# janosh/torch-mnf

Measured on NVIDIA B200. Metric: flow log-prob points/s, higher is better.
Workload: dtype f32

## Files before the change

torch-mnf_b200/csrc/flow_pl.cu:

```cuda
#include "flow_math.cuh"
#include "tc_common.cuh"

namespace mnf {
namespace fpl {
using tc::smem_u32; using tc::mbar_init; using tc::mbar_arrive; using tc::mbar_wait; using tc::bulk_load;

constexpr int PMAX = 511;
constexpr int BP_FLOATS = 512;
constexpr int MAX_GROUPS = 2 * MNF_MAX_OPS;
constexpr int HDR_INTS = 4;
constexpr int HDR_FLOATS = MAX_GROUPS * HDR_INTS;
constexpr int MAX_H = 64;
constexpr double FAST_T = 32.0;
constexpr float FAST_B_MAX = 32.f;
constexpr int NB_MIN = 64, NB_MAX = 2048;
constexpr int SMEM_TABLE_FLOATS = 216 * 1024 / 4;
constexpr double LOG2E_D = 1.4426950408889634;

__host__ __device__ constexpr int round4i(int n) { return (n + 3) / 4 * 4; }
__host__ __device__ constexpr int nsf_doff(int K) { return 4 * K; }
__host__ __device__ constexpr int nsf_org(int K) { return 4 * K + round4i(2 * (K - 1)); }
__host__ __device__ constexpr int nsf_stride4(int K) { return (nsf_org(K) / 4 + 1) | 1; }
constexpr int AFF_ORG = 4, AFF_STRIDE4 = 3;
__host__ __device__ constexpr int region_floats(int stride4) { return BP_FLOATS + (PMAX + 1) * 4 * stride4; }

struct GroupList {
    int n;
    int region[MAX_GROUPS];
    unsigned char op[MAX_GROUPS];
    unsigned char which[MAX_GROUPS];
    signed char group_of[MNF_MAX_OPS][2];
};

__device__ __forceinline__ int bucket_of(float c, float lo, float inv, float nbm1) {
    const float t = fminf(fmaxf((c - lo) * inv, 0.f), nbm1);
    return __float_as_int(__fadd_rz(t, 8388608.f)) & 0x7fffff;
}

constexpr int BW = 8;

__device__ int envelope_line(const double *A, const double *B, int o0, int K, double lo, double hi) {
    int l = o0;
    if (lo == -INFINITY || hi == INFINITY) {
        const double sg = lo == -INFINITY ? -1.0 : 1.0;
        for (int k = o0 + 1; k < o0 + K; ++k)
            if (sg * A[k] > sg * A[l] || (A[k] == A[l] && B[k] > B[l])) l = k;
    } else {
        const double m = 0.5 * lo + 0.5 * hi;
        for (int k = o0 + 1; k < o0 + K; ++k)
            if (fma(A[k], m, B[k]) > fma(A[l], m, B[l])) l = k;
    }
    return l;
}

__device__ double envelope_gap(const double *A, const double *B, int K, double lo, double hi, double e) {
    double g = 0.0;
    for (int o0 = 0; o0 < 2 * K; o0 += K) {
        const int l = envelope_line(A, B, o0, K, lo, hi);
        const double vl = fma(A[l], e, B[l]);
        for (int k = o0; k < o0 + K; ++k) g = fmax(g, fma(A[k], e, B[k]) - vl);
    }
    return g;
}

__device__ bool split_piece(const double *A, const double *B, int K, double lo, double hi, double *out, int *cnt) {
    const double TN = FAST_T / LOG2E_D;
    auto emit = [&](double s) {
        const int p = atomicAdd(cnt, 1);
        if (p < PMAX) out[p] = s;
        return p < PMAX;
    };
    double seg[2][2] = {{lo, hi}, {0.0, 0.0}};
    int nseg = 1;
    if (lo == -INFINITY && hi == INFINITY) {
        if (!emit(0.0)) return false;
        seg[0][1] = 0.0, seg[1][0] = 0.0, seg[1][1] = INFINITY, nseg = 2;
    }
    for (int q = 0; q < nseg; ++q) {
        double a = seg[q][0], b = seg[q][1];
        const bool left = a == -INFINITY, right = b == INFINITY;
        if (left || right) {
            const double e = left ? b : a;
            if (envelope_gap(A, B, K, a, b, e) <= TN) continue;
            double w = fmax(1.0, fabs(e)), s;
            for (;;) {
                s = (double)(float)(left ? e - w : e + w);
                if (fabs(s) > 1.0e38) return false;
                if (envelope_gap(A, B, K, left ? -INFINITY : s, left ? s : INFINITY, s) <= TN) break;
                w *= 2.0;
            }
            if (!emit(s)) return false;
            a = left ? s : e, b = left ? e : s;
        }
        double st[64][2];
        int sp = 0;
        st[sp][0] = a, st[sp][1] = b, ++sp;
        while (sp) {
            --sp;
            const double x0 = st[sp][0], x1 = st[sp][1];
            if (envelope_gap(A, B, K, x0, x1, x0) <= TN && envelope_gap(A, B, K, x0, x1, x1) <= TN) continue;
            const double s = (double)(float)(0.5 * x0 + 0.5 * x1);
            if (!(s > x0 && s < x1) || sp + 2 > 64 || !emit(s)) return false;
            st[sp][0] = s, st[sp][1] = x1, ++sp;
            st[sp][0] = x0, st[sp][1] = s, ++sp;
        }
    }
    return true;
}

__device__ __forceinline__ double piece_point(const double *bp, int n, int i, double &lo, double &hi) {
    lo = i > 0 ? bp[i - 1] : -INFINITY;
    hi = i < n ? bp[i] : INFINITY;
    if (n == 0) return 0.0;
    if (i == 0) return hi - 1.0 - fabs(hi);
    if (i == n) return lo + 1.0 + fabs(lo);
    return 0.5 * lo + 0.5 * hi;
}

__device__ int net_pre_maps(const float *__restrict__ net, const int *sizes, int upto, double m, double (*va)[MNF_MAX_HIDDEN],
                            double (*vb)[MNF_MAX_HIDDEN], int lane) {
    const double slope_neg = (double)0.2f;
    int cur = 0;
    if (lane == 0) va[0][0] = 1.0, vb[0][0] = 0.0;
    __syncwarp();
    const float *p = net;
    for (int t = 0; t <= upto; ++t) {
        const int n_in = sizes[t], n_out = sizes[t + 1];
        const float *bias = p + n_in * n_out;
        for (int k = lane; k < n_out; k += 32) {
            double A = 0.0, B = (double)bias[k];
            const float *w = p + (size_t)k * n_in;
            for (int j = 0; j < n_in; ++j) {
                const double wj = (double)w[j];
                A = fma(wj, va[cur][j], A);
                B = fma(wj, vb[cur][j], B);
            }
            if (t < upto) {
                const double s = fma(A, m, B) > 0.0 ? 1.0 : slope_neg;
                A *= s, B *= s;
            }
            va[cur ^ 1][k] = A, vb[cur ^ 1][k] = B;
        }
        __syncwarp();
        cur ^= 1;
        p += n_in * n_out + n_out;
    }
    return cur;
}

__global__ void __launch_bounds__(32 * BW) flow_pl_build_kernel(const __grid_constant__ FlowProgram prog, const __grid_constant__ GroupList gl,
                                                                const float *__restrict__ params, float *__restrict__ image) {
    __shared__ double s_bp[512], s_tmp[512];
    __shared__ double s_va[BW][2][MNF_MAX_HIDDEN], s_vb[BW][2][MNF_MAX_HIDDEN];
    __shared__ int s_bidx[PMAX];
    __shared__ int s_n, s_ncand, s_fail;
    const int g = blockIdx.x, tid = threadIdx.x, warp = tid >> 5, lane = tid & 31, nt = blockDim.x;
    auto sort_bp = [&](int tot) {
        for (int e = tid; e < tot; e += nt) {
            const double v = s_bp[e];
            int r = 0;
            for (int u = 0; u < tot; ++u) r += (s_bp[u] < v || (s_bp[u] == v && u < e)) ? 1 : 0;
            s_tmp[r] = v;
        }
        __syncthreads();
        for (int e = tid; e < tot; e += nt) s_bp[e] = s_tmp[e];
        __syncthreads();
    };
    const mnf_flow_op &op = prog.ops[gl.op[g]];
    const bool nsf = op.type == MNF_OP_NSF_CL;
    const int K = op.K, L = op.n_lin, n_out = op.sizes[L];
    int n_nets = 0, net_off[2], net_slot[2];
    if (nsf) {
        net_off[0] = op.net_off[gl.which[g]], net_slot[0] = 0, n_nets = 1;
    } else {
        if (op.flags & MNF_FLAG_SCALE) net_off[n_nets] = op.net_off[0], net_slot[n_nets++] = 0;
        if (op.flags & MNF_FLAG_SHIFT) net_off[n_nets] = op.net_off[1], net_slot[n_nets++] = 1;
    }
    if (tid == 0) s_n = 0, s_ncand = 0;
    __syncthreads();

    bool over = false;
    for (int l = 1; l < L; ++l) {
        const int n = s_n;
        for (int i = warp; i <= n; i += BW) {
            double lo, hi;
            const double m = piece_point(s_bp, n, i, lo, hi);
            for (int q = 0; q < n_nets; ++q) {
                const int cur = net_pre_maps(params + net_off[q], op.sizes, l - 1, m, s_va[warp], s_vb[warp], lane);
                for (int k = lane; k < op.sizes[l]; k += 32) {
                    const double a = s_va[warp][cur][k], b = s_vb[warp][cur][k];
                    if (a != 0.0) {
                        const double tz = -b / a;
                        if (tz > lo && tz < hi && fabs(tz) < 3.0e38) {
                            const int pos = atomicAdd(&s_ncand, 1);
                            if (pos < 512) s_tmp[pos] = tz;
                        }
                    }
                }
                __syncwarp();
            }
        }
        __syncthreads();
        const int nc = s_ncand, tot = n + nc;
        if (tot > PMAX) {
            over = true;
            break;
        }
        for (int e = tid; e < nc; e += nt) s_bp[n + e] = s_tmp[e];
        __syncthreads();
        sort_bp(tot);
        if (tid == 0) s_n = tot, s_ncand = 0;
        __syncthreads();
    }

    float *region = image + gl.region[g];
    int *hdr = reinterpret_cast<int *>(image) + g * HDR_INTS;
    const int n = over ? 0 : s_n;
    if (tid == 0) hdr[0] = n, hdr[1] = over ? 1 : 0, hdr[2] = 0, hdr[3] = 0;
    for (int e = tid; e < BP_FLOATS; e += nt) region[e] = e < n ? (float)s_bp[e] : INFINITY;
    if (over) return;
    const int stride = 4 * (nsf ? nsf_stride4(K) : AFF_STRIDE4);
    auto write_rows = [&](int nn, float *rows, bool fast) {
        for (int i = warp; i <= nn; i += BW) {
            double lo, hi;
            const double m = piece_point(s_bp, nn, i, lo, hi);
            const float org = nn == 0 ? 0.f : (float)(i == 0 ? s_bp[0] : s_bp[i - 1]);
            float *row = rows + (size_t)i * stride;
            for (int e = lane; e < stride; e += 32) row[e] = 0.f;
            __syncwarp();
            for (int q = 0; q < n_nets; ++q) {
                const int cur = net_pre_maps(params + net_off[q], op.sizes, L - 1, m, s_va[warp], s_vb[warp], lane);
                const double *va = s_va[warp][cur], *vb = s_vb[warp][cur];
                for (int o = lane; o < n_out; o += 32) {
                    double A = va[o], B = vb[o], sc = 1.0;
                    if (fast && nsf) {
                        sc = LOG2E_D;
                        if (o < 2 * K) {
                            const int l = envelope_line(va, vb, o < K ? 0 : K, K, lo, hi);
                            A -= va[l], B -= vb[l];
                        }
                    }
                    const double V = fma(A, (double)org, B);
                    int ia, iv;
                    if (!nsf) ia = net_slot[q], iv = 2 + net_slot[q];
                    else if (o < 2 * K) ia = 4 * (o >> 1) + (o & 1), iv = ia + 2;
                    else ia = nsf_doff(K) + 2 * (o - 2 * K), iv = ia + 1;
                    row[ia] = (float)(A * sc), row[iv] = (float)(V * sc);
                }
                __syncwarp();
            }
            if (lane == 0) row[nsf ? nsf_org(K) : AFF_ORG] = org;
        }
    };
    write_rows(n, region + BP_FLOATS, false);

    __syncthreads();
    if (tid == 0) s_ncand = 0, s_fail = nsf && !(op.bound <= FAST_B_MAX);
    __syncthreads();
    if (nsf && !s_fail) {
        for (int i = warp; i <= n; i += BW) {
            double lo, hi;
            const double m = piece_point(s_bp, n, i, lo, hi);
            const int cur = net_pre_maps(params + net_off[0], op.sizes, L - 1, m, s_va[warp], s_vb[warp], lane);
            if (lane == 0 && !split_piece(s_va[warp][cur], s_vb[warp][cur], K, lo, hi, s_tmp, &s_ncand)) s_fail = 1;
            __syncwarp();
        }
    }
    __syncthreads();
    const int nf = n + s_ncand;
    if (s_fail || nf > PMAX) return;
    for (int e = tid; e < nf - n; e += nt) s_bp[n + e] = s_tmp[e];
    __syncthreads();
    sort_bp(nf);
    const int fast_off = BP_FLOATS + (n + 1) * stride, rows_floats = (nf + 1) * stride;
    const int budget = min((PMAX - n) * stride, SMEM_TABLE_FLOATS / gl.n);
    int nb = NB_MIN;
    float lo32 = 0.f, inv = 0.f;
    for (bool found = false; !found; nb *= 2) {
        if (nb > NB_MAX || 4 + 4 * nb + rows_floats > budget) return;
        for (int ab = 0; ab < 9 && !found; ++ab) {
            const int a = ab / 3, b = ab % 3;
            if (nf && a + b >= nf) continue;
            lo32 = nf ? (float)s_bp[a] : 0.f;
            const float hi32 = nf ? (float)s_bp[nf - 1 - b] : 0.f;
            inv = hi32 > lo32 ? (float)((double)nb / ((double)hi32 - (double)lo32)) : 0.f;
            for (int e = tid; e < nf; e += nt) s_bidx[e] = bucket_of((float)s_bp[e], lo32, inv, (float)(nb - 1));
            __syncthreads();
            int bad = 0;
            for (int e = tid; e + 3 < nf; e += nt) bad |= s_bidx[e] == s_bidx[e + 3];
            found = !__syncthreads_or(bad);
        }
        if (found) break;
    }
    float *fast = region + fast_off;
    for (int j = tid; j < nb; j += nt) {
        int a = 0, b = nf;
        while (a < b) {
            const int mid = (a + b) >> 1;
            if (s_bidx[mid] < j) a = mid + 1; else b = mid;
        }
        float4 r;
        r.x = __int_as_float(a);
        r.y = a < nf && s_bidx[a] == j ? (float)s_bp[a] : INFINITY;
        r.z = a + 1 < nf && s_bidx[a + 1] == j ? (float)s_bp[a + 1] : INFINITY;
        r.w = a + 2 < nf && s_bidx[a + 2] == j ? (float)s_bp[a + 2] : INFINITY;
        reinterpret_cast<float4 *>(fast)[1 + j] = r;
    }
    if (tid == 0) {
        fast[0] = lo32, fast[1] = inv, fast[2] = (float)(nb - 1), fast[3] = __int_as_float(4 + 4 * nb);
        hdr[2] = fast_off, hdr[3] = 4 + 4 * nb + rows_floats;
    }
    write_rows(nf, fast + 4 + 4 * nb, true);
}

struct Params {
    FlowProgram prog;
    GroupList gl;
    const float *params, *x, *image;
    float *y, *log_det, *base_lp, *inter;
    long long n_rows;
    int dir_flags, smem_floats;
    mnf_gather_out gather;
};

__device__ __forceinline__ float2 f2_fma(float2 a, float2 b, float2 c) {
    unsigned long long ra = *reinterpret_cast<unsigned long long *>(&a), rb = *reinterpret_cast<unsigned long long *>(&b),
                       rc = *reinterpret_cast<unsigned long long *>(&c), rd;
    asm("fma.rn.f32x2 %0, %1, %2, %3;" : "=l"(rd) : "l"(ra), "l"(rb), "l"(rc));
    return *reinterpret_cast<float2 *>(&rd);
}

__device__ __noinline__ void mlp_fp32(const float *__restrict__ net, int n_lin, const int *sizes, float c, float *out) {
    float h[2][MAX_H];
    h[0][0] = c;
    int cur = 0;
    const float *p = net;
    for (int t = 0; t < n_lin; ++t) {
        const int n_in = sizes[t], n_o = sizes[t + 1];
        for (int k = 0; k < n_o; ++k) {
            float acc = p[n_in * n_o + k];
            for (int j = 0; j < n_in; ++j) acc = fmaf(p[k * n_in + j], h[cur][j], acc);
            if (t + 1 < n_lin) h[cur ^ 1][k] = leaky02(acc);
            else out[k] = acc;
        }
        cur ^= 1;
        p += n_in * n_o + n_o;
    }
}

template <int K>
__device__ __noinline__ float2 nsf_fallback(const float *__restrict__ net, int n_lin, const int *sizes, float B, float edge_deriv, float c,
                                            bool inverse, float tr) {
    float raw[3 * K - 1], ld = 0.f;
    mlp_fp32(net, n_lin, sizes, c, raw);
    rq_spline<K, true>(raw, K, B, edge_deriv, inverse, tr, ld);
    return make_float2(tr, ld);
}
__device__ __noinline__ float mlp_fp32_scalar(const float *__restrict__ net, int n_lin, const int *sizes, float c) {
    float out[1];
    mlp_fp32(net, n_lin, sizes, c, out);
    return out[0];
}

template <int S>
__device__ __forceinline__ void search_steps(uint32_t &a, float c) {
    float t;
    asm("ld.shared.f32 %0, [%1+%2];" : "=f"(t) : "r"(a), "n"(4 * (S - 1)));
    if (c > t) a += 4u * S;
    if constexpr (S > 1) search_steps<S / 2>(a, c);
}

template <bool SM>
__device__ __forceinline__ int find_piece(const float *tb, float c) {
    if constexpr (SM) {
        const uint32_t base = smem_u32(tb);
        uint32_t a = base;
        search_steps<(PMAX + 1) / 2>(a, c);
        return (int)((a - base) >> 2);
    } else {
        int pos = 0;
#pragma unroll
        for (int s = (PMAX + 1) / 2; s >= 1; s >>= 1) pos += (c > tb[pos + s - 1]) ? s : 0;
        return pos;
    }
}

enum { KIND_PLAIN = 0, KIND_FAST = 1, KIND_OVER = 2 };

template <bool SM>
__device__ __forceinline__ const float4 *piece_row(const float *tb, bool fast, float c, int stride4) {
    if (fast) {
        const float4 gr = *reinterpret_cast<const float4 *>(tb);
        const float4 bk = reinterpret_cast<const float4 *>(tb)[1 + bucket_of(c, gr.x, gr.y, gr.z)];
        const int piece = __float_as_int(bk.x) + (c > bk.y) + (c > bk.z) + (c > bk.w);
        return reinterpret_cast<const float4 *>(tb + __float_as_int(gr.w)) + piece * stride4;
    }
    return reinterpret_cast<const float4 *>(tb + BP_FLOATS) + find_piece<SM>(tb, c) * stride4;
}

__device__ __forceinline__ float ex2_approx(float x) {
    float r;
    asm("ex2.approx.ftz.f32 %0, %1;" : "=f"(r) : "f"(x));
    return r;
}
__device__ __forceinline__ float sqrt_approx(float x) {
    float r;
    asm("sqrt.approx.ftz.f32 %0, %1;" : "=f"(r) : "f"(x));
    return r;
}
__device__ __forceinline__ float lg2_approx(float x) {
    float r;
    asm("lg2.approx.ftz.f32 %0, %1;" : "=f"(r) : "f"(x));
    return r;
}

constexpr float LOG2E = 1.4426950408889634f, LN2 = 0.6931471805599453f;

template <int K, bool FAST>
__device__ __forceinline__ void unit_knots(const float *raw, float twoB, float *tw, float *th) {
    constexpr float span = 1.f - kMinBin * (float)K;
    float ew[K], eh[K], sw = 0.f, sh = 0.f, scw, sch, offw, offh;
    if constexpr (FAST) {
#pragma unroll
        for (int k = 0; k < K; ++k) {
            ew[k] = ex2_approx(raw[k]), eh[k] = ex2_approx(raw[K + k]);
            sw += ew[k], sh += eh[k];
        }
        const float r = frcp<true>(sw * sh), s = twoB * LOG2E;
        scw = s * (r * sh), sch = s * (r * sw);
        offw = offh = -0.5f * s;
    } else {
        float mw = raw[0], mh = raw[K];
#pragma unroll
        for (int k = 1; k < K; ++k) mw = fmaxf(mw, raw[k]), mh = fmaxf(mh, raw[K + k]);
        const float mwn = -mw * LOG2E, mhn = -mh * LOG2E;
#pragma unroll
        for (int k = 0; k < K; ++k) {
            ew[k] = ex2_approx(fmaf(raw[k], LOG2E, mwn)), eh[k] = ex2_approx(fmaf(raw[K + k], LOG2E, mhn));
            sw += ew[k], sh += eh[k];
        }
        scw = twoB * frcp<true>(sw) * LOG2E, sch = twoB * frcp<true>(sh) * LOG2E;
        offw = twoB > 80.f ? -scw : 0.f, offh = twoB > 80.f ? -sch : 0.f;
    }
    float pw = 0.f, ph = 0.f;
#pragma unroll
    for (int k = 0; k < K; ++k) {
        pw += ex2_approx(fmaf(ew[k], scw, offw)), ph += ex2_approx(fmaf(eh[k], sch, offh));
        ew[k] = pw, eh[k] = ph;
    }
    float c1w, c1h;
    if constexpr (FAST) {
        const float r = frcp<true>(pw * ph);
        c1w = 2.f * span * (r * ph), c1h = 2.f * span * (r * pw);
    } else {
        c1w = 2.f * span * frcp<true>(pw), c1h = 2.f * span * frcp<true>(ph);
    }
    tw[0] = th[0] = -1.f;
#pragma unroll
    for (int k = 0; k + 1 < K; ++k) {
        tw[k + 1] = fmaf(ew[k], c1w, -1.f + 2.f * (float)(k + 1) * kMinBin);
        th[k + 1] = fmaf(eh[k], c1h, -1.f + 2.f * (float)(k + 1) * kMinBin);
    }
    tw[K] = th[K] = 1.f;
}

__device__ __forceinline__ float knot_derivative_log2(float r) {
    return fmaf(LN2, r > 20.f * LOG2E ? r : lg2_approx(2.f + ex2_approx(r)), kMinDeriv);
}

template <int K, bool FAST, class DerivFn>
__device__ __forceinline__ void rq_spline_lazy(const float *raw, float B, float inv_B, float edge_deriv, bool inverse, float &v, float &ld,
                                               DerivFn deriv) {
    float cw[K + 1], ch[K + 1];
    unit_knots<K, FAST>(raw, 2.f * B, cw, ch);
    const float u = v * inv_B;
    const float *sk = inverse ? ch : cw;
    int idx = 0;
    float xk = cw[0], xk1 = cw[1], yk = ch[0], yk1 = ch[1];
#pragma unroll
    for (int k = 1; k < K; ++k) {
        const bool ge = u >= sk[k];
        idx += ge ? 1 : 0;
        xk = ge ? cw[k] : xk, xk1 = ge ? cw[k + 1] : xk1;
        yk = ge ? ch[k] : yk, yk1 = ge ? ch[k + 1] : yk1;
    }
    const float wk = xk1 - xk, hk = yk1 - yk;
    const float r0 = deriv(max(idx - 1, 0)), r1 = deriv(min(idx, K - 2));
    float dk, dk1;
    if constexpr (FAST) {
        dk = (idx > 0) ? knot_derivative_log2(r0) : edge_deriv;
        dk1 = (idx < K - 1) ? knot_derivative_log2(r1) : edge_deriv;
    } else {
        dk = (idx > 0) ? knot_derivative<true>(r0) : edge_deriv;
        dk1 = (idx < K - 1) ? knot_derivative<true>(r1) : edge_deriv;
    }
    if (inverse) {
        const float dkw = dk * wk, dk1w = dk1 * wk;
        const float dsw = dkw + dk1w - 2.f * hk;
        const float dy = u - yk;
        const float a = dy * dsw + hk * (hk - dkw);
        const float b = hk * dkw - dy * dsw;
        const float c = -hk * dy;
        const float disc = fmaxf(b * b - 4.f * a * c, 0.f);
        const float root = __fdividef(2.f * c, -b - sqrt_approx(disc));
        v = (root * wk + xk) * B;
        const float tt = root * (1.f - root);
        const float omr = 1.f - root;
        const float den = wk * (hk + dsw * tt);
        const float num = (hk * hk) * wk * (dk1w * (root * root) + 2.f * hk * tt + dkw * (omr * omr));
        const float rd = frcp<true>(den);
        ld -= __logf(num * rd * rd);
    } else {
        const float sk_ = __fdividef(hk, wk);
        const float dsum = dk + dk1 - 2.f * sk_;
        const float th = __fdividef(u - xk, wk);
        const float tt = th * (1.f - th);
        const float numer = hk * (sk_ * (th * th) + dk * tt);
        const float den = sk_ + dsum * tt;
        const float omt = 1.f - th;
        const float num = (sk_ * sk_) * (dk1 * (th * th) + 2.f * sk_ * tt + dk * (omt * omt));
        const float rd = frcp<true>(den);
        v = fmaf(numer, rd, yk) * B;
        ld += __logf(num * rd * rd);
    }
}

constexpr int THREADS = 1024;

struct Exec {
    int type;
    int k;
    int g0, g1;
    int flag;
    int pad[3];
    float c[8];
};
static_assert(sizeof(Exec) == 64, "two 16-byte rows of ints, two of floats");

__device__ __forceinline__ void build_exec(const Params &p, Exec *ex, int *n_exec, int lane) {
    const int n = p.prog.n_ops, inverse = p.dir_flags & 1;
    if (lane < n) {
        const int k = inverse ? n - 1 - lane : lane;
        const mnf_flow_op &op = p.prog.ops[k];
        Exec e{};
        e.k = k;
        if (op.type == MNF_OP_AFFINE_CONST) {
            const double s0 = p.params[op.aux_off], s1 = p.params[op.aux_off + 1];
            const double t0 = p.params[op.aux_off + 2], t1 = p.params[op.aux_off + 3];
            if (inverse) {
                const double e0 = exp(-s0), e1 = exp(-s1);
                e.c[0] = (float)e0, e.c[3] = (float)e1, e.c[4] = (float)(-t0 * e0), e.c[5] = (float)(-t1 * e1), e.c[6] = (float)(-(s0 + s1));
            } else {
                e.c[0] = (float)exp(s0), e.c[3] = (float)exp(s1), e.c[4] = (float)t0, e.c[5] = (float)t1, e.c[6] = (float)(s0 + s1);
            }
        } else if (op.type == MNF_OP_GLOW) {
            const float *W = p.params + op.aux_off + (inverse ? 4 : 0);
            e.c[0] = W[0], e.c[1] = W[1], e.c[2] = W[2], e.c[3] = W[3];
            e.c[6] = inverse ? -p.params[op.aux_off + 8] : p.params[op.aux_off + 8];
        } else if (op.type == MNF_OP_AFFINE_HALF) {
            e.type = 1, e.g0 = p.gl.group_of[k][0], e.flag = (op.flags & MNF_FLAG_PARITY) ? 1 : 0;
        } else {
            e.type = 2, e.flag = inverse ? 0 : 1;
            e.g0 = p.gl.group_of[k][inverse ? 1 : 0], e.g1 = p.gl.group_of[k][inverse ? 0 : 1];
            e.c[0] = op.bound, e.c[1] = 1.f / op.bound, e.c[2] = op.edge_deriv;
        }
        ex[lane] = e;
    }
    __syncwarp();
    if (lane == 0) {
        int j = 0;
        bool open = false;
        double M[4], b[2], ld;
        for (int i = 0; i < n; ++i) {
            const Exec e = ex[i];
            if (e.type != 0 || p.inter) {
                ex[j++] = e, open = false;
                continue;
            }
            if (!open) {
                for (int q = 0; q < 4; ++q) M[q] = e.c[q];
                b[0] = e.c[4], b[1] = e.c[5], ld = e.c[6];
                ++j, open = true;
            } else {
                const double W0 = e.c[0], W1 = e.c[1], W2 = e.c[2], W3 = e.c[3];
                const double n00 = M[0] * W0 + M[1] * W2, n01 = M[0] * W1 + M[1] * W3;
                const double n10 = M[2] * W0 + M[3] * W2, n11 = M[2] * W1 + M[3] * W3;
                const double nb0 = b[0] * W0 + b[1] * W2 + e.c[4], nb1 = b[0] * W1 + b[1] * W3 + e.c[5];
                M[0] = n00, M[1] = n01, M[2] = n10, M[3] = n11, b[0] = nb0, b[1] = nb1, ld += e.c[6];
            }
            Exec f{};
            for (int q = 0; q < 4; ++q) f.c[q] = (float)M[q];
            f.c[4] = (float)b[0], f.c[5] = (float)b[1], f.c[6] = (float)ld;
            ex[j - 1] = f;
        }
        *n_exec = j;
    }
}

template <int K, bool SM>
__device__ __forceinline__ void run_points(const Params &p, const float *smem, const int *s_off, const int *s_goff, const int *s_kind,
                                           const Exec *ex, int n_exec) {
    const bool sum_lp = p.dir_flags & 2;
    auto table = [&](int g) -> const float * {
        if constexpr (SM) return smem + s_off[g];
        const int o = s_off[g];
        return o >= 0 ? smem + o : p.image + s_goff[g];
    };
    const long long stride = (long long)gridDim.x * blockDim.x;
#pragma unroll 1
    for (long long r = (long long)blockIdx.x * blockDim.x + threadIdx.x; r < p.n_rows; r += stride) {
        float v0, v1, ld = 0.f;
        {
            const float2 xin = ld_stream2(reinterpret_cast<const float2 *>(p.x) + r);
            v0 = xin.x, v1 = xin.y;
        }
#pragma unroll 1
        for (int kk = 0; kk < n_exec; ++kk) {
            const int4 ei = *reinterpret_cast<const int4 *>(&ex[kk]);
            if (ei.x == 0) {
                const float4 m = *reinterpret_cast<const float4 *>(ex[kk].c), b = *reinterpret_cast<const float4 *>(ex[kk].c + 4);
                const float n0 = fmaf(v1, m.z, fmaf(v0, m.x, b.x)), n1 = fmaf(v1, m.w, fmaf(v0, m.y, b.y));
                v0 = n0, v1 = n1, ld += b.z;
            } else if (ei.x == 1) {
                const mnf_flow_op &op = p.prog.ops[ei.y];
                const bool parity = ex[kk].flag != 0;
                const float c = parity ? v1 : v0;
                float tr = parity ? v0 : v1;
                const int g = ei.z;
                float s = 0.f, t = 0.f;
                if (g < 0) {
                } else if (s_kind[g] != KIND_OVER) {
                    const float4 *row = piece_row<SM>(table(g), s_kind[g] == KIND_FAST, c, AFF_STRIDE4);
                    const float4 q = row[0];
                    const float d = c - row[1].x;
                    s = fmaf(q.x, d, q.z), t = fmaf(q.y, d, q.w);
                } else {
                    if (op.flags & MNF_FLAG_SCALE) s = mlp_fp32_scalar(p.params + op.net_off[0], op.n_lin, op.sizes, c);
                    if (op.flags & MNF_FLAG_SHIFT) t = mlp_fp32_scalar(p.params + op.net_off[1], op.n_lin, op.sizes, c);
                }
                if (p.dir_flags & 1) {
                    tr = (tr - t) / expf(s), ld -= s;
                } else {
                    tr = expf(s) * tr + t, ld += s;
                }
                if (parity) v0 = tr; else v1 = tr;
            } else {
                const float4 cs = *reinterpret_cast<const float4 *>(ex[kk].c);
                const bool first_f1 = ex[kk].flag != 0;
#pragma unroll 1
                for (int step = 0; step < 2; ++step) {
                    const bool use_f1 = (step == 0) == first_f1;
                    const float c = use_f1 ? v0 : v1;
                    float tr = use_f1 ? v1 : v0;
                    const float B = cs.x;
                    if (tr >= -B && tr <= B) {
                        const int g = step ? ei.w : ei.z;
                        const int kind = s_kind[g];
                        if (kind != KIND_OVER) {
                            const float4 *row = piece_row<SM>(table(g), kind == KIND_FAST, c, nsf_stride4(K));
                            const float d = c - row[nsf_org(K) / 4].x;
                            const float2 dd = make_float2(d, d);
                            float raw[2 * K];
#pragma unroll
                            for (int j = 0; j < K; ++j) {
                                const float4 q = row[j];
                                const float2 o = f2_fma(make_float2(q.x, q.y), dd, make_float2(q.z, q.w));
                                raw[2 * j] = o.x, raw[2 * j + 1] = o.y;
                            }
                            const float2 *dv = reinterpret_cast<const float2 *>(row) + nsf_doff(K) / 2;
                            const auto deriv = [&](int j) {
                                const float2 q = dv[j];
                                return fmaf(q.x, d, q.y);
                            };
                            if (kind == KIND_FAST) rq_spline_lazy<K, true>(raw, B, cs.y, cs.z, (p.dir_flags & 1) != 0, tr, ld, deriv);
                            else rq_spline_lazy<K, false>(raw, B, cs.y, cs.z, (p.dir_flags & 1) != 0, tr, ld, deriv);
                        } else {
                            const mnf_flow_op &op = p.prog.ops[ei.y];
                            const float2 o = nsf_fallback<K>(p.params + op.net_off[use_f1 ? 0 : 1], op.n_lin, op.sizes, B, cs.z, c,
                                                             (p.dir_flags & 1) != 0, tr);
                            tr = o.x, ld += o.y;
                        }
                        if (use_f1) v1 = tr; else v0 = tr;
                    }
                }
            }
            if (p.inter) st_stream2(reinterpret_cast<float2 *>(p.inter + ((size_t)kk * p.n_rows + r) * 2), make_float2(v0, v1));
        }
        float lp = fmaf(-0.5f, fmaf(v0, v0, v1 * v1), -1.8378770664093453f);
        if (sum_lp) lp += ld;
        if (p.y) st_stream2(reinterpret_cast<float2 *>(p.y) + r, make_float2(v0, v1));
        if (p.log_det) p.log_det[r] = ld;
        if (p.base_lp) p.base_lp[r] = lp;
        if (p.gather.multicast_ptr) {
            asm volatile("multimem.st.relaxed.sys.global.f32 [%0], %1;" ::"l"(p.gather.multicast_ptr + p.gather.row_offset + r), "f"(lp)
                         : "memory");
        } else {
            for (int g = 0; g < p.gather.n_peers; ++g) p.gather.peer_ptrs[g][p.gather.row_offset + r] = lp;
        }
    }
}

template <int K>
__global__ void __launch_bounds__(THREADS, 1) flow_pl_kernel(const __grid_constant__ Params p) {
    extern __shared__ __align__(16) float smem[];
    __shared__ __align__(16) Exec s_exec[MNF_MAX_OPS];
    __shared__ int s_off[MAX_GROUPS], s_goff[MAX_GROUPS], s_kind[MAX_GROUPS];
    __shared__ int s_allfit, s_nexec;
    __shared__ __align__(8) unsigned long long s_bar;
    const int lane = threadIdx.x & 31, ng = p.gl.n;
    const uint32_t bar = smem_u32(&s_bar);
    if (threadIdx.x == 0) {
        mbar_init(bar, 1);
        asm volatile("fence.mbarrier_init.release.cluster;" ::: "memory");
    }
    __syncthreads();
    if (threadIdx.x >= 32 && threadIdx.x < 64) build_exec(p, s_exec, &s_nexec, lane);
    if (threadIdx.x < 32) {
        const int *hdr = reinterpret_cast<const int *>(p.image);
        int total = 0, fit = 1;
        for (int base = 0; base < ng; base += 32) {
            const int g = base + lane;
            int sz = 0, ov = 0, src = 0;
            if (g < ng) {
                const int4 h = *reinterpret_cast<const int4 *>(hdr + g * HDR_INTS);
                const int s4 = p.prog.ops[p.gl.op[g]].type == MNF_OP_NSF_CL ? nsf_stride4(K) : AFF_STRIDE4;
                ov = h.y;
                src = p.gl.region[g] + h.z;
                sz = ov ? 0 : h.z ? h.w : BP_FLOATS + (h.x + 1) * 4 * s4;
                s_kind[g] = ov ? KIND_OVER : h.z ? KIND_FAST : KIND_PLAIN;
                s_goff[g] = src;
            }
            int inc = sz;
#pragma unroll
            for (int o = 1; o < 32; o <<= 1) {
                const int t = __shfl_up_sync(0xffffffffu, inc, o);
                if (lane >= o) inc += t;
            }
            const int off = total + inc - sz;
            const bool ok = off + sz <= p.smem_floats;
            if (g < ng) {
                s_off[g] = (ov || !ok) ? -1 : off;
                if (!ov && ok) {
                    asm volatile("mbarrier.expect_tx.relaxed.cta.shared::cta.b64 [%0], %1;" ::"r"(bar), "r"((uint32_t)sz * 4u) : "memory");
                    bulk_load(smem_u32(smem + off), p.image + src, (uint32_t)sz * 4u, bar);
                }
            }
            fit &= __all_sync(0xffffffffu, g >= ng || ov || ok) ? 1 : 0;
            total += __shfl_sync(0xffffffffu, inc, 31);
        }
        __syncwarp();
        if (lane == 0) {
            s_allfit = fit;
            mbar_arrive(bar);
        }
    }
    __syncthreads();
    mbar_wait(bar, 0);
    if (s_allfit) run_points<K, true>(p, smem, s_off, s_goff, s_kind, s_exec, s_nexec);
    else run_points<K, false>(p, smem, s_off, s_goff, s_kind, s_exec, s_nexec);
}

#define MNF_PL_BINS(X) X(4) X(5) X(6) X(8) X(10) X(12) X(16)
constexpr int K_MAX = 16;
static bool k_instantiated(int K) {
#define MNF_PL_HAVE(KK) if (K == KK) return true;
    MNF_PL_BINS(MNF_PL_HAVE)
#undef MNF_PL_HAVE
    return false;
}

struct Plan {
    bool ok = false;
    int K = 8;
    GroupList gl;
    int64_t image_floats = 0;
};

static Plan make_plan(const mnf_flow_op *ops, int n_ops, int dim) {
    Plan pl;
    if (dim != 2 || n_ops < 1 || n_ops > MNF_MAX_OPS) return pl;
    int K = 0, n = 0;
    int64_t off = HDR_FLOATS;
    for (int k = 0; k < n_ops; ++k) {
        const mnf_flow_op &op = ops[k];
        pl.gl.group_of[k][0] = pl.gl.group_of[k][1] = -1;
        if (op.type == MNF_OP_AFFINE_CONST || op.type == MNF_OP_GLOW) continue;
        if (op.type != MNF_OP_AFFINE_HALF && op.type != MNF_OP_NSF_CL) return pl;
        if (op.n_lin < 2 || op.n_lin > MNF_MAX_LIN || op.sizes[0] != 1) return pl;
        for (int l = 1; l < op.n_lin; ++l)
            if (op.sizes[l] < 1 || op.sizes[l] > MAX_H) return pl;
        if (op.type == MNF_OP_NSF_CL) {
            if (!k_instantiated(op.K)) return pl;
            if (K && op.K != K) return pl;
            K = op.K;
            if (op.sizes[op.n_lin] != 3 * K - 1) return pl;
            for (int which = 0; which < 2; ++which) {
                pl.gl.group_of[k][which] = (signed char)n;
                pl.gl.op[n] = (unsigned char)k, pl.gl.which[n] = (unsigned char)which, pl.gl.region[n] = (int)off;
                off += region_floats(nsf_stride4(K));
                ++n;
            }
        } else {
            if (op.sizes[op.n_lin] != 1) return pl;
            if (!(op.flags & (MNF_FLAG_SCALE | MNF_FLAG_SHIFT))) continue;
            pl.gl.group_of[k][0] = (signed char)n;
            pl.gl.op[n] = (unsigned char)k, pl.gl.which[n] = 0, pl.gl.region[n] = (int)off;
            off += region_floats(AFF_STRIDE4);
            ++n;
        }
    }
    if (n == 0) return pl;
    pl.gl.n = n;
    pl.K = K ? K : 8;
    pl.image_floats = off;
    pl.ok = true;
    return pl;
}

template <int K>
static int launch_k(const Params &p, const DeviceProps *dp, size_t smem_bytes, cudaStream_t st) {
    static thread_local size_t attr_set[64] = {};
    int dev = 0;
    MNF_CUDA(cudaGetDevice(&dev));
    if (dev < 0 || dev >= 64 || attr_set[dev] < smem_bytes) {
        MNF_CUDA(cudaFuncSetAttribute(flow_pl_kernel<K>, cudaFuncAttributeMaxDynamicSharedMemorySize, (int)smem_bytes));
        if (dev >= 0 && dev < 64) attr_set[dev] = smem_bytes;
    }
    const int threads = p.n_rows <= (long long)dp->sm_count * 64 ? 64 : p.n_rows <= (long long)dp->sm_count * 256 ? 256 : THREADS;
    long long blocks = (p.n_rows + threads - 1) / threads;
    if (blocks > dp->sm_count) blocks = dp->sm_count;
    flow_pl_kernel<K><<<(unsigned)blocks, threads, smem_bytes, st>>>(p);
    return launch_status("flow_pl_kernel");
}

}

int64_t flow_pl_workspace_floats(int n_ops) {
    if (n_ops < 1) n_ops = 1;
    if (n_ops > MNF_MAX_OPS) n_ops = MNF_MAX_OPS;
    return fpl::HDR_FLOATS + (int64_t)2 * n_ops * fpl::region_floats(fpl::nsf_stride4(fpl::K_MAX));
}

int64_t flow_pl_image_floats(const mnf_flow_op *ops, int n_ops, int dim) {
    const fpl::Plan pl = fpl::make_plan(ops, n_ops, dim);
    return pl.ok ? pl.image_floats : 0;
}

int flow_pl_build(const mnf_flow_op *ops, int n_ops, const float *params, int dim, float *image, cudaStream_t stream) {
    using namespace fpl;
    const Plan pl = make_plan(ops, n_ops, dim);
    MNF_REQUIRE(pl.ok, MNF_E_SHAPE, "program has no piecewise-linear form");
    MNF_REQUIRE(params && image && ((uintptr_t)image % 16) == 0, MNF_E_ARG, "NULL or misaligned pointer");
    FlowProgram prog;
    prog.n_ops = n_ops;
    for (int k = 0; k < n_ops; ++k) prog.ops[k] = ops[k];
    flow_pl_build_kernel<<<pl.gl.n, 32 * BW, 0, stream>>>(prog, pl.gl, params, image);
    return launch_status("flow_pl_build_kernel");
}

int launch_flow_pl(const mnf_flow_op *ops, int n_ops, const float *params, const float *x, float *y, float *log_det,
                   float *base_lp, float *inter, int64_t n_rows, int dim, int dir_flags, float *workspace,
                   const mnf_gather_out *gather, cudaStream_t stream, bool plan_only) {
    using namespace fpl;
    const Plan pl = make_plan(ops, n_ops, dim);
    if (!pl.ok) return 1;
    if (plan_only) return 0;
    if (!workspace) return 1;
    const DeviceProps *dp = device_props();
    MNF_REQUIRE(dp != nullptr, MNF_E_DEVICE, "no CUDA device");
    MNF_REQUIRE(((uintptr_t)workspace % 16) == 0, MNF_E_ALIGN, "workspace must be 16-byte aligned");
    MNF_REQUIRE(((uintptr_t)x % 8) == 0 && (!y || ((uintptr_t)y % 8) == 0) && (!inter || ((uintptr_t)inter % 8) == 0), MNF_E_ALIGN,
                "x, y and intermediates must be 8-byte aligned");
    MNF_REQUIRE(n_rows > 0, MNF_E_ARG, "bad row count");
    if (!(dir_flags & 4)) {
        const int rc = flow_pl_build(ops, n_ops, params, dim, workspace, stream);
        if (rc) return rc;
    }
    Params p{};
    p.prog.n_ops = n_ops;
    for (int k = 0; k < n_ops; ++k) p.prog.ops[k] = ops[k];
    p.gl = pl.gl;
    p.params = params, p.x = x, p.image = workspace, p.y = y, p.log_det = log_det, p.base_lp = base_lp, p.inter = inter;
    p.n_rows = n_rows, p.dir_flags = dir_flags & 3;
    if (gather) {
        MNF_REQUIRE(gather->n_peers >= 0 && gather->n_peers <= MNF_MAX_PEERS, MNF_E_ARG, "bad n_peers");
        p.gather = *gather;
    }
    size_t want = (size_t)(pl.image_floats - HDR_FLOATS) * sizeof(float);
    const size_t cap = (size_t)dp->smem_optin - 4096;
    if (want > cap) want = cap;
    want &= ~(size_t)15;
    p.smem_floats = (int)(want / sizeof(float));
#define MNF_PL_LAUNCH(KK) if (pl.K == KK) return launch_k<KK>(p, dp, want, stream);
    MNF_PL_BINS(MNF_PL_LAUNCH)
#undef MNF_PL_LAUNCH
    return 1;
}

}
```

Measured before the change: 12.61 billion.

## Pack spline knot math into f32x2, defer log-det logs, template on direction

Reworks the rational-quadratic spline: width and height knot accumulation now uses paired f32x2 add/fma, and only the needed knot pair is reconstructed from cumulative sums instead of materialising full knot arrays. Per-spline log calls are replaced by a running mantissa/exponent product that is flushed with a single lg2 at the end or before fallback paths. Divisions become reciprocal multiplies, and the inverse flag becomes a template parameter so each kernel variant is specialised. This cuts MUFU and ALU work per point, at the cost of doubling kernel instantiations and a slight change in numeric rounding.

```diff
diff --git a/torch-mnf_b200/csrc/flow_pl.cu b/torch-mnf_b200/csrc/flow_pl.cu
--- a/torch-mnf_b200/csrc/flow_pl.cu
+++ b/torch-mnf_b200/csrc/flow_pl.cu
@@ -329,6 +329,12 @@
     asm("fma.rn.f32x2 %0, %1, %2, %3;" : "=l"(rd) : "l"(ra), "l"(rb), "l"(rc));
     return *reinterpret_cast<float2 *>(&rd);
 }
+__device__ __forceinline__ float2 f2_add(float2 a, float2 b) {
+    unsigned long long ra = *reinterpret_cast<unsigned long long *>(&a), rb = *reinterpret_cast<unsigned long long *>(&b), rd;
+    asm("add.rn.f32x2 %0, %1, %2;" : "=l"(rd) : "l"(ra), "l"(rb));
+    return *reinterpret_cast<float2 *>(&rd);
+}
+__device__ __forceinline__ float2 f2_splat(float a) { return make_float2(a, a); }
 
 __device__ __noinline__ void mlp_fp32(const float *__restrict__ net, int n_lin, const int *sizes, float c, float *out) {
     float h[2][MAX_H];
@@ -416,74 +422,87 @@
 
 constexpr float LOG2E = 1.4426950408889634f, LN2 = 0.6931471805599453f;
 
+__device__ __forceinline__ float knot_const(float k) { return fmaf(2.f * kMinBin, k, -1.f); }
+
 template <int K, bool FAST>
-__device__ __forceinline__ void unit_knots(const float *raw, float twoB, float *tw, float *th) {
+__device__ __forceinline__ void unit_knots(const float *raw, float twoB, float2 *S, float2 &c1) {
     constexpr float span = 1.f - kMinBin * (float)K;
-    float ew[K], eh[K], sw = 0.f, sh = 0.f, scw, sch, offw, offh;
+    float2 e[K], sc, off;
     if constexpr (FAST) {
+        float2 s1;
 #pragma unroll
         for (int k = 0; k < K; ++k) {
-            ew[k] = ex2_approx(raw[k]), eh[k] = ex2_approx(raw[K + k]);
-            sw += ew[k], sh += eh[k];
-        }
-        const float r = frcp<true>(sw * sh), s = twoB * LOG2E;
-        scw = s * (r * sh), sch = s * (r * sw);
-        offw = offh = -0.5f * s;
+            e[k] = make_float2(ex2_approx(raw[k]), ex2_approx(raw[K + k]));
+            s1 = k ? f2_add(s1, e[k]) : e[k];
+        }
+        const float r = frcp<true>(s1.x * s1.y), s = twoB * LOG2E;
+        sc = make_float2(s * (r * s1.y), s * (r * s1.x));
+        off = f2_splat(-0.5f * s);
     } else {
-        float mw = raw[0], mh = raw[K];
+        float mw = raw[0], mh = raw[K], sw = 0.f, sh = 0.f;
 #pragma unroll
         for (int k = 1; k < K; ++k) mw = fmaxf(mw, raw[k]), mh = fmaxf(mh, raw[K + k]);
         const float mwn = -mw * LOG2E, mhn = -mh * LOG2E;
 #pragma unroll
         for (int k = 0; k < K; ++k) {
-            ew[k] = ex2_approx(fmaf(raw[k], LOG2E, mwn)), eh[k] = ex2_approx(fmaf(raw[K + k], LOG2E, mhn));
-            sw += ew[k], sh += eh[k];
-        }
-        scw = twoB * frcp<true>(sw) * LOG2E, sch = twoB * frcp<true>(sh) * LOG2E;
-        offw = twoB > 80.f ? -scw : 0.f, offh = twoB > 80.f ? -sch : 0.f;
-    }
-    float pw = 0.f, ph = 0.f;
+            e[k] = make_float2(ex2_approx(fmaf(raw[k], LOG2E, mwn)), ex2_approx(fmaf(raw[K + k], LOG2E, mhn)));
+            sw += e[k].x, sh += e[k].y;
+        }
+        sc = make_float2(twoB * frcp<true>(sw) * LOG2E, twoB * frcp<true>(sh) * LOG2E);
+        off = make_float2(twoB > 80.f ? -sc.x : 0.f, twoB > 80.f ? -sc.y : 0.f);
+    }
+    float2 p;
 #pragma unroll
     for (int k = 0; k < K; ++k) {
-        pw += ex2_approx(fmaf(ew[k], scw, offw)), ph += ex2_approx(fmaf(eh[k], sch, offh));
-        ew[k] = pw, eh[k] = ph;
-    }
-    float c1w, c1h;
+        const float2 a = f2_fma(e[k], sc, off);
+        const float2 x = make_float2(ex2_approx(a.x), ex2_approx(a.y));
+        p = k ? f2_add(p, x) : x;
+        if (k + 1 < K) S[k] = p;
+    }
     if constexpr (FAST) {
-        const float r = frcp<true>(pw * ph);
-        c1w = 2.f * span * (r * ph), c1h = 2.f * span * (r * pw);
+        const float r = frcp<true>(p.x * p.y);
+        c1 = make_float2(2.f * span * (r * p.y), 2.f * span * (r * p.x));
     } else {
-        c1w = 2.f * span * frcp<true>(pw), c1h = 2.f * span * frcp<true>(ph);
-    }
-    tw[0] = th[0] = -1.f;
-#pragma unroll
-    for (int k = 0; k + 1 < K; ++k) {
-        tw[k + 1] = fmaf(ew[k], c1w, -1.f + 2.f * (float)(k + 1) * kMinBin);
-        th[k + 1] = fmaf(eh[k], c1h, -1.f + 2.f * (float)(k + 1) * kMinBin);
-    }
-    tw[K] = th[K] = 1.f;
+        c1 = make_float2(2.f * span * frcp<true>(p.x), 2.f * span * frcp<true>(p.y));
+    }
 }
 
 __device__ __forceinline__ float knot_derivative_log2(float r) {
     return fmaf(LN2, r > 20.f * LOG2E ? r : lg2_approx(2.f + ex2_approx(r)), kMinDeriv);
 }
 
-template <int K, bool FAST, class DerivFn>
-__device__ __forceinline__ void rq_spline_lazy(const float *raw, float B, float inv_B, float edge_deriv, bool inverse, float &v, float &ld,
+__device__ __forceinline__ void ld_mul(float &P, int &E, float q) {
+    P *= q;
+    const int eb = __float_as_int(P) & 0x7f800000;
+    E += (eb >> 23) - 127;
+    P *= __int_as_float(0x7f000000 - eb);
+}
+template <bool INV>
+__device__ __forceinline__ void ld_flush(float &ld, float &P, int &E) {
+    ld = fmaf(INV ? -LN2 : LN2, lg2_approx(P) + (float)E, ld);
+    P = 1.f, E = 0;
+}
+
+template <int K, bool FAST, bool INV, class DerivFn>
+__device__ __forceinline__ void rq_spline_lazy(const float *raw, float B, float inv_B, float edge_deriv, float &v, float &P, int &E,
                                                DerivFn deriv) {
-    float cw[K + 1], ch[K + 1];
-    unit_knots<K, FAST>(raw, 2.f * B, cw, ch);
+    float2 S[K - 1], c1;
+    unit_knots<K, FAST>(raw, 2.f * B, S, c1);
     const float u = v * inv_B;
-    const float *sk = inverse ? ch : cw;
     int idx = 0;
-    float xk = cw[0], xk1 = cw[1], yk = ch[0], yk1 = ch[1];
+    float2 lo = f2_splat(0.f), hi = S[0];
 #pragma unroll
     for (int k = 1; k < K; ++k) {
-        const bool ge = u >= sk[k];
+        const bool ge = u >= fmaf(INV ? S[k - 1].y : S[k - 1].x, INV ? c1.y : c1.x, knot_const((float)k));
         idx += ge ? 1 : 0;
-        xk = ge ? cw[k] : xk, xk1 = ge ? cw[k + 1] : xk1;
-        yk = ge ? ch[k] : yk, yk1 = ge ? ch[k + 1] : yk1;
-    }
+        lo = ge ? S[k - 1] : lo;
+        if (k + 1 < K) hi = ge ? S[k] : hi;
+    }
+    const float fidx = __int_as_float(0x4b000000 | idx) - 8388608.f;
+    const float k0 = knot_const(fidx), k1 = knot_const(fidx + 1.f);
+    const float xk = fmaf(lo.x, c1.x, k0), yk = fmaf(lo.y, c1.y, k0);
+    const bool last = idx == K - 1;
+    const float xk1 = last ? 1.f : fmaf(hi.x, c1.x, k1), yk1 = last ? 1.f : fmaf(hi.y, c1.y, k1);
     const float wk = xk1 - xk, hk = yk1 - yk;
     const float r0 = deriv(max(idx - 1, 0)), r1 = deriv(min(idx, K - 2));
     float dk, dk1;
@@ -494,7 +513,7 @@
         dk = (idx > 0) ? knot_derivative<true>(r0) : edge_deriv;
         dk1 = (idx < K - 1) ? knot_derivative<true>(r1) : edge_deriv;
     }
-    if (inverse) {
+    if constexpr (INV) {
         const float dkw = dk * wk, dk1w = dk1 * wk;
         const float dsw = dkw + dk1w - 2.f * hk;
         const float dy = u - yk;
@@ -502,18 +521,19 @@
         const float b = hk * dkw - dy * dsw;
         const float c = -hk * dy;
         const float disc = fmaxf(b * b - 4.f * a * c, 0.f);
-        const float root = __fdividef(2.f * c, -b - sqrt_approx(disc));
+        const float root = 2.f * c * frcp<true>(-b - sqrt_approx(disc));
         v = (root * wk + xk) * B;
         const float tt = root * (1.f - root);
         const float omr = 1.f - root;
         const float den = wk * (hk + dsw * tt);
         const float num = (hk * hk) * wk * (dk1w * (root * root) + 2.f * hk * tt + dkw * (omr * omr));
         const float rd = frcp<true>(den);
-        ld -= __logf(num * rd * rd);
+        ld_mul(P, E, num * rd * rd);
     } else {
-        const float sk_ = __fdividef(hk, wk);
+        const float rw = frcp<true>(wk);
+        const float sk_ = hk * rw;
         const float dsum = dk + dk1 - 2.f * sk_;
-        const float th = __fdividef(u - xk, wk);
+        const float th = (u - xk) * rw;
         const float tt = th * (1.f - th);
         const float numer = hk * (sk_ * (th * th) + dk * tt);
         const float den = sk_ + dsum * tt;
@@ -521,7 +541,7 @@
         const float num = (sk_ * sk_) * (dk1 * (th * th) + 2.f * sk_ * tt + dk * (omt * omt));
         const float rd = frcp<true>(den);
         v = fmaf(numer, rd, yk) * B;
-        ld += __logf(num * rd * rd);
+        ld_mul(P, E, num * rd * rd);
     }
 }
 
@@ -597,7 +617,7 @@
     }
 }
 
-template <int K, bool SM>
+template <int K, bool SM, bool INV>
 __device__ __forceinline__ void run_points(const Params &p, const float *smem, const int *s_off, const int *s_goff, const int *s_kind,
                                            const Exec *ex, int n_exec) {
     const bool sum_lp = p.dir_flags & 2;
@@ -609,7 +629,8 @@
     const long long stride = (long long)gridDim.x * blockDim.x;
 #pragma unroll 1
     for (long long r = (long long)blockIdx.x * blockDim.x + threadIdx.x; r < p.n_rows; r += stride) {
-        float v0, v1, ld = 0.f;
+        float v0, v1, ld = 0.f, P = 1.f;
+        int E = 0;
         {
             const float2 xin = ld_stream2(reinterpret_cast<const float2 *>(p.x) + r);
             v0 = xin.x, v1 = xin.y;
@@ -635,10 +656,11 @@
                     const float d = c - row[1].x;
                     s = fmaf(q.x, d, q.z), t = fmaf(q.y, d, q.w);
                 } else {
+                    ld_flush<INV>(ld, P, E);
                     if (op.flags & MNF_FLAG_SCALE) s = mlp_fp32_scalar(p.params + op.net_off[0], op.n_lin, op.sizes, c);
                     if (op.flags & MNF_FLAG_SHIFT) t = mlp_fp32_scalar(p.params + op.net_off[1], op.n_lin, op.sizes, c);
                 }
-                if (p.dir_flags & 1) {
+                if constexpr (INV) {
                     tr = (tr - t) / expf(s), ld -= s;
                 } else {
                     tr = expf(s) * tr + t, ld += s;
@@ -672,12 +694,13 @@
                                 const float2 q = dv[j];
                                 return fmaf(q.x, d, q.y);
                             };
-                            if (kind == KIND_FAST) rq_spline_lazy<K, true>(raw, B, cs.y, cs.z, (p.dir_flags & 1) != 0, tr, ld, deriv);
-                            else rq_spline_lazy<K, false>(raw, B, cs.y, cs.z, (p.dir_flags & 1) != 0, tr, ld, deriv);
+                            if (kind == KIND_FAST) rq_spline_lazy<K, true, INV>(raw, B, cs.y, cs.z, tr, P, E, deriv);
+                            else rq_spline_lazy<K, false, INV>(raw, B, cs.y, cs.z, tr, P, E, deriv);
                         } else {
                             const mnf_flow_op &op = p.prog.ops[ei.y];
+                            ld_flush<INV>(ld, P, E);
                             const float2 o = nsf_fallback<K>(p.params + op.net_off[use_f1 ? 0 : 1], op.n_lin, op.sizes, B, cs.z, c,
-                                                             (p.dir_flags & 1) != 0, tr);
+                                                             INV, tr);
                             tr = o.x, ld += o.y;
                         }
                         if (use_f1) v1 = tr; else v0 = tr;
@@ -686,6 +709,7 @@
             }
             if (p.inter) st_stream2(reinterpret_cast<float2 *>(p.inter + ((size_t)kk * p.n_rows + r) * 2), make_float2(v0, v1));
         }
+        ld_flush<INV>(ld, P, E);
         float lp = fmaf(-0.5f, fmaf(v0, v0, v1 * v1), -1.8378770664093453f);
         if (sum_lp) lp += ld;
         if (p.y) st_stream2(reinterpret_cast<float2 *>(p.y) + r, make_float2(v0, v1));
@@ -700,7 +724,7 @@
     }
 }
 
-template <int K>
+template <int K, bool INV>
 __global__ void __launch_bounds__(THREADS, 1) flow_pl_kernel(const __grid_constant__ Params p) {
     extern __shared__ __align__(16) float smem[];
     __shared__ __align__(16) Exec s_exec[MNF_MAX_OPS];
@@ -756,8 +780,8 @@
     }
     __syncthreads();
     mbar_wait(bar, 0);
-    if (s_allfit) run_points<K, true>(p, smem, s_off, s_goff, s_kind, s_exec, s_nexec);
-    else run_points<K, false>(p, smem, s_off, s_goff, s_kind, s_exec, s_nexec);
+    if (s_allfit) run_points<K, true, INV>(p, smem, s_off, s_goff, s_kind, s_exec, s_nexec);
+    else run_points<K, false, INV>(p, smem, s_off, s_goff, s_kind, s_exec, s_nexec);
 }
 
 #define MNF_PL_BINS(X) X(4) X(5) X(6) X(8) X(10) X(12) X(16)
@@ -817,19 +841,19 @@
     return pl;
 }
 
-template <int K>
+template <int K, bool INV>
 static int launch_k(const Params &p, const DeviceProps *dp, size_t smem_bytes, cudaStream_t st) {
     static thread_local size_t attr_set[64] = {};
     int dev = 0;
     MNF_CUDA(cudaGetDevice(&dev));
     if (dev < 0 || dev >= 64 || attr_set[dev] < smem_bytes) {
-        MNF_CUDA(cudaFuncSetAttribute(flow_pl_kernel<K>, cudaFuncAttributeMaxDynamicSharedMemorySize, (int)smem_bytes));
+        MNF_CUDA(cudaFuncSetAttribute(flow_pl_kernel<K, INV>, cudaFuncAttributeMaxDynamicSharedMemorySize, (int)smem_bytes));
         if (dev >= 0 && dev < 64) attr_set[dev] = smem_bytes;
     }
     const int threads = p.n_rows <= (long long)dp->sm_count * 64 ? 64 : p.n_rows <= (long long)dp->sm_count * 256 ? 256 : THREADS;
     long long blocks = (p.n_rows + threads - 1) / threads;
     if (blocks > dp->sm_count) blocks = dp->sm_count;
-    flow_pl_kernel<K><<<(unsigned)blocks, threads, smem_bytes, st>>>(p);
+    flow_pl_kernel<K, INV><<<(unsigned)blocks, threads, smem_bytes, st>>>(p);
     return launch_status("flow_pl_kernel");
 }
 
@@ -891,7 +915,8 @@
     if (want > cap) want = cap;
     want &= ~(size_t)15;
     p.smem_floats = (int)(want / sizeof(float));
-#define MNF_PL_LAUNCH(KK) if (pl.K == KK) return launch_k<KK>(p, dp, want, stream);
+#define MNF_PL_LAUNCH(KK) \
+    if (pl.K == KK) return (dir_flags & 1) ? launch_k<KK, true>(p, dp, want, stream) : launch_k<KK, false>(p, dp, want, stream);
     MNF_PL_BINS(MNF_PL_LAUNCH)
 #undef MNF_PL_LAUNCH
     return 1;
```

Measured after the change: 13.49 billion, median of 6. 7.0% higher.
